# iamwinter/UMPR

Hardware: AMD Instinct MI355X
Metric: training samples/sec (higher is better)
Workload: dtype f32

## Files before the change

### umpr_amd/csrc/conv3x3.hip

```cpp
#include "umpr_common.h"
#include "umpr_internal.h"
#include "umpr_tiles.h"
#include <stdlib.h>
#include <type_traits>

namespace {

struct ConvParams {
  const float* x;
  const float* wm;
  const float* bias;
  const float* mask;
  float* y;
  int N, C, H, W, Cout, relu;
  long p0_base;
  long p_end;
};

template <int TM, int TN, bool BIAS, bool MASK, bool TAIL>
__device__ __forceinline__ void igemm_epilogue_as(const f32x16 (&tot)[TM][TN], const ConvParams& p, int HW, int row0,
                                                  const long (&obase)[TN], const bool (&pv)[TN]) {
  const int Cout = p.Cout;
  const bool relu = p.relu != 0;
  float bv[TM][16];
// ... 306 lines not shown
    okb = (okb & ~(1u << v)) | ((unsigned)ok << v);
  };
  auto store_a = [&](int v, int buf) {
    float* S = As[buf] + adst[v];
    S[0] = ra[v].x; S[LDA] = ra[v].y; S[2 * LDA] = ra[v].z; S[3 * LDA] = ra[v].w;
  };
  auto store_b = [&](int v, int buf) {
    const bool ok = (okb >> v) & 1;
    float* S = Ps[buf] + bdst[v];
    if (VEC == 4) *reinterpret_cast<float4*>(S) = ok ? rb[v] : make_float4(0.f, 0.f, 0.f, 0.f);
    else *reinterpret_cast<float2*>(S) = ok ? make_float2(rb[v].x, rb[v].y) : make_float2(0.f, 0.f);
  };
  constexpr int NPIECE = AV + BV;
  constexpr int KS = KC / 2;
  constexpr int ST0 = KS - NPIECE;
  static_assert(2 * NPIECE <= KS, "staging pieces must fit the k-steps of one stage");

#pragma unroll
  for (int v = 0; v < AV; ++v) load_a(v, 0);
#pragma unroll
  for (int v = 0; v < BV; ++v) load_b(v, 0);
#pragma unroll
  for (int v = 0; v < AV; ++v) store_a(v, 0);
#pragma unroll
  for (int v = 0; v < BV; ++v) store_b(v, 0);
  __syncthreads();
  for (int s0 = 0; s0 < ns; s0 += SFLUSH) {
#pragma unroll
    for (int i = 0; i < TM; ++i)
#pragma unroll
      for (int j = 0; j < TN; ++j)
#pragma unroll
        for (int r = 0; r < 16; ++r) acc[i][j][r] = 0.f;
    const int s1 = min(ns, s0 + SFLUSH);
    for (int s = s0; s < s1; ++s) {
      const int cur = s & 1;
      const int sn = min(s + 1, ns - 1);
      const float* as = As[cur] + half * LDA + wm * WTM + l31;
      const float* ps = Ps[cur];
      float a[2][TM], b[2][TN];
#pragma unroll
      for (int i = 0; i < TM; ++i) a[0][i] = as[i * 32];
#pragma unroll
      for (int j = 0; j < TN; ++j) b[0][j] = ps[boff[j]];
#pragma unroll
      for (int kk = 0; kk < KS; ++kk) {
        const int cb = kk & 1, nb = cb ^ 1;
        const int k1 = kk + 1, cl = k1 / 9, tap = k1 % 9;
#pragma unroll
        for (int m = 0; m < TM * TN; ++m) {
          const int i = m / TN, j = m % TN;
          acc[i][j] = mfma32(a[cb][i], b[cb][j], acc[i][j]);
          if (m == 0 && kk + 1 < KS) {
#pragma unroll
            for (int ii = 0; ii < TM; ++ii) a[nb][ii] = as[2 * k1 * LDA + ii * 32];
          }
          if (m == (TM * TN > 1 ? 1 : 0) && kk + 1 < KS) {
#pragma unroll
            for (int jj = 0; jj < TN; ++jj) b[nb][jj] = ps[boff[jj] + cl * PLANE + (tap / 3) * RW + (tap % 3)];
          }
          if (m == TM * TN - 1) {
            if (kk < AV) load_a(kk, sn);
            else if (kk < NPIECE) load_b(kk - AV, sn);
            else if (kk >= ST0 && kk - ST0 < AV) store_a(kk - ST0, cur ^ 1);
            else if (kk >= ST0 + AV) store_b(kk - ST0 - AV, cur ^ 1);
          }
          __builtin_amdgcn_sched_barrier(0);
        }
      }
      __syncthreads();
    }
#pragma unroll
    for (int i = 0; i < TM; ++i)
#pragma unroll
      for (int j = 0; j < TN; ++j) tot[i][j] += acc[i][j];
  }

  long obase[TN];
  bool pv[TN];
#pragma unroll
  for (int j = 0; j < TN; ++j) {
    const int d = wn * WTN + j * 32 + l31;
    pv[j] = d <= dlast;
    const int loc = yx0 + min(d, dlast);
    const int dn = loc / HW;
    obase[j] = (long)(n0 + dn) * p.Cout * HW + (loc - dn * HW);
  }
  igemm_epilogue<TM, TN>(tot, p, HW, m0 + __builtin_amdgcn_readfirstlane(wm) * WTM, half, obase, pv);
}

__global__ void pack_weights_kernel(const float* __restrict__ w, float* __restrict__ wp, int M, int C, int CinW,
                                    int transposed) {
  const int ns = (C + V2_CC - 1) / V2_CC;
  const long total = (long)M * ns * V2_KC;
  for (long i = blockIdx.x * (long)blockDim.x + threadIdx.x; i < total; i += (long)gridDim.x * blockDim.x) {
    const int kq = (int)(i % V2_KC);
    const long r = i / V2_KC;
    const int s = (int)(r % ns), m = (int)(r / ns);
    const int hf = kq & 1, j = kq >> 1;
    const int cl = j / 9, tap = j - cl * 9;
    const int c = s * V2_CC + cl + 2 * hf;
    float v = 0.f;
    if (c < C) v = transposed ? w[((long)c * CinW + m) * 9 + 8 - tap] : w[((long)m * CinW + c) * 9 + tap];
    wp[i] = v;
  }
}

constexpr int kSlots128 = 512;
template <int W>
void launch_v2(ConvParams p, int bn, hipStream_t s) {
  const long NP = (long)p.N * p.H * p.W;
  p.p0_base = 0; p.p_end = NP;
  if (p.Cout <= 64) {
    if (W >= 224 && bn != 128 && bn != 64) {
      const long ptiles = cdiv(NP, 256);
      dim3 grid((unsigned)(cdiv(ptiles, 8) * 8 * cdiv(p.Cout, 64)));
      conv3x3_igemm_v2_kernel<64, 256, W><<<grid, 256, 0, s>>>(p);
      return;
    }
    const long ptiles = cdiv(NP, 128);
    dim3 grid((unsigned)(cdiv(ptiles, 8) * 8 * cdiv(p.Cout, 64)));
    conv3x3_igemm_v2_kernel<64, 128, W><<<grid, 256, 0, s>>>(p);
    return;
  }
  const int mt = cdiv(p.Cout, 128);
  const long pt = cdiv(NP, 128);
  long pt_main = pt;
  if (bn == 64) pt_main = 0;
  else if (bn == 0 && pt * mt > kSlots128) {
    const long full = (pt * mt / kSlots128) * kSlots128;
    if (pt * mt - full > 0 && pt * mt - full <= kSlots128 * 3 / 4) pt_main = full / mt;
  }
  if (pt_main > 0) {
    ConvParams q = p;
    q.p_end = pt_main * 128 < NP ? pt_main * 128 : NP;
    dim3 grid((unsigned)(cdiv(pt_main, 8) * 8 * mt));
    conv3x3_igemm_v2_kernel<128, 128, W><<<grid, 256, 0, s>>>(q);
  }
  if (pt_main < pt) {
    ConvParams q = p;
    q.p0_base = pt_main * 128;
    dim3 grid((unsigned)(cdiv(cdiv(NP - q.p0_base, 64), 8) * 8 * mt));
    conv3x3_igemm_v2_kernel<128, 64, W><<<grid, 256, 0, s>>>(q);
  }
}

__global__ void flip_transpose_kernel(const float* __restrict__ w, float* __restrict__ wt, int Cout, int Cin) {
  const long total = (long)Cout * Cin * 9;
  for (long i = blockIdx.x * (long)blockDim.x + threadIdx.x; i < total; i += (long)gridDim.x * blockDim.x) {
    const int t = (int)(i % 9);
    const long r = i / 9;
    const int co = (int)(r % Cout), ci = (int)(r / Cout);
    wt[i] = w[((long)co * Cin + ci) * 9 + (8 - t)];
  }
}

struct WgradParams {
  const float* gz;
  const float* x;
  float* slab;
  float* bslab;
  int N, Cin, Cout, H, W;
  int R, CW;
  int segs_y, segs_x, nsegs, segs_per_split;
};

constexpr int WG_LDG = 33;
constexpr int WG_PLMAX = 103;

__global__ __launch_bounds__(256) void conv3x3_wgrad_kernel(WgradParams p) {
  __shared__ float Gs[2][64 * WG_LDG];
  __shared__ float Xs[2][64 * WG_PLMAX];
  __shared__ int pxoff[32];
  const int tid = threadIdx.x, lane = tid & 63, wave = tid >> 6;
  const int wm = wave >> 1, wn = wave & 1;
  const int l31 = lane & 31, kh = lane >> 5;
  const int co0 = blockIdx.y * 64, ci0 = blockIdx.x * 64;
  const int split = blockIdx.z;
  const int RW = p.CW + 2;
  const int patch = (p.R + 2) * RW;
  const int PL = patch | 1;
  const int npx = p.R * p.CW;
  const int HW = p.H * p.W;
  if (tid < 32) pxoff[tid] = tid < npx ? (tid / p.CW) * RW + (tid % p.CW) : 0;

  f32x16 acc[9];
#pragma unroll
  for (int t = 0; t < 9; ++t)
#pragma unroll
    for (int r = 0; r < 16; ++r) acc[t][r] = 0.f;
  float bsum[8];
#pragma unroll
  for (int v = 0; v < 8; ++v) bsum[v] = 0.f;

  const int sbeg = split * p.segs_per_split;
  const int send = min(p.nsegs, sbeg + p.segs_per_split);
  const int xs_total = 64 * patch;
  constexpr int XV = (64 * 102 + 255) / 256;
  float rg[8];
  float rx[XV];
  unsigned okg = 0, okx = 0;

  auto load = [&](int seg) {
    okg = 0; okx = 0;
    const int sx = seg % p.segs_x;
    const int sy = (seg / p.segs_x) % p.segs_y;
    const int n = seg / (p.segs_x * p.segs_y);
    const int y0 = sy * p.R, x0 = sx * p.CW;
#pragma unroll
    for (int v = 0; v < 8; ++v) {
      const int e = tid + v * 256;
      const int co = e >> 5, px = e & 31;
      const int r = px / p.CW, c = px - r * p.CW;
      const bool ok = px < npx && co0 + co < p.Cout && y0 + r < p.H && x0 + c < p.W;
      rg[v] = p.gz[ok ? ((long)n * p.Cout + co0 + co) * HW + (y0 + r) * p.W + x0 + c : 0];
      okg |= (unsigned)ok << v;
    }
#pragma unroll
    for (int v = 0; v < XV; ++v) {
      const int e = tid + v * 256;
      const int ci = e / patch, q = e - ci * patch;
      const int rr = q / RW, cc = q - rr * RW;
      const int yy = y0 - 1 + rr, xx = x0 - 1 + cc;
      const bool ok = e < xs_total && ci0 + ci < p.Cin && yy >= 0 && yy < p.H && xx >= 0 && xx < p.W;
      rx[v] = p.x[ok ? ((long)n * p.Cin + ci0 + ci) * HW + yy * p.W + xx : 0];
      okx |= (unsigned)ok << v;
    }
  };
  auto store = [&](int buf) {
#pragma unroll
    for (int v = 0; v < 8; ++v) {
      const int e = tid + v * 256;
      const float gv = ((okg >> v) & 1) ? rg[v] : 0.f;
      Gs[buf][(e >> 5) * WG_LDG + (e & 31)] = gv;
      if (p.bslab && blockIdx.x == 0) bsum[v] += gv;
    }
#pragma unroll
    for (int v = 0; v < XV; ++v) {
      const int e = tid + v * 256;
      if (e < xs_total) {
        const int ci = e / patch, q = e - ci * patch;
        Xs[buf][ci * PL + q] = ((okx >> v) & 1) ? rx[v] : 0.f;
      }
    }
  };

  if (sbeg < send) {
    load(sbeg);
    store(0);
  }
  __syncthreads();
  for (int s = sbeg; s < send; ++s) {
    const int cur = (s - sbeg) & 1;
    if (s + 1 < send) load(s + 1);
    const float* gs = Gs[cur] + (wm * 32 + l31) * WG_LDG;
    const float* xs = Xs[cur] + (wn * 32 + l31) * PL;
    float a[2], b[2][9];
    {
      a[0] = gs[kh];
      const float* xp = xs + pxoff[kh];
#pragma unroll
      for (int t = 0; t < 9; ++t) b[0][t] = xp[(t / 3) * RW + (t % 3)];
    }
#pragma unroll
    for (int kk = 0; kk < 16; ++kk) {
      const int cb = kk & 1, nb = cb ^ 1;
      if (kk + 1 < 16) {
        const int px = 2 * (kk + 1) + kh;
        a[nb] = gs[px];
        const float* xp = xs + pxoff[px];
#pragma unroll
        for (int t = 0; t < 9; ++t) b[nb][t] = xp[(t / 3) * RW + (t % 3)];
      }
      __builtin_amdgcn_sched_barrier(0);
#pragma unroll
      for (int t = 0; t < 9; ++t) acc[t] = mfma32(a[cb], b[cb][t], acc[t]);
      __builtin_amdgcn_sched_barrier(0);
    }
    if (s + 1 < send) store(cur ^ 1);
    __syncthreads();
  }

#pragma unroll
  for (int t = 0; t < 9; ++t) {
#pragma unroll
    for (int r = 0; r < 16; ++r) {
      const int co = co0 + wm * 32 + mfma_row(r, lane);
      const int ci = ci0 + wn * 32 + l31;
      if (co < p.Cout && ci < p.Cin) p.slab[(((long)split * 9 + t) * p.Cout + co) * p.Cin + ci] = acc[t][r];
    }
  }
  if (p.bslab && blockIdx.x == 0) {
#pragma unroll
    for (int v = 0; v < 8; ++v) {
      float sv = bsum[v];
#pragma unroll
      for (int o = 16; o > 0; o >>= 1) sv += __shfl_xor(sv, o, 64);
      const int co = co0 + (tid >> 5) + 8 * v;
      if ((tid & 31) == 0 && co < p.Cout) p.bslab[(long)split * p.Cout + co] = sv;
    }
  }
}

template <int R, int CW>
__global__ __launch_bounds__(256, 2) void conv3x3_wgrad_v2_kernel(WgradParams p) {
  constexpr int RW = CW + 2, PP = (R + 2) * RW, PL = PP | 1, NPX = R * CW;
  constexpr int G = 256 / PP;
  constexpr int CPG = (64 + G - 1) / G;
  static_assert((CW & 1) == 0 && NPX <= 32 && PP <= 102, "segment geometry");
  __shared__ float Gs[2][64 * WG_LDG];
  __shared__ float Xs[2][64 * PL];
  const int tid = threadIdx.x, lane = tid & 63, wave = tid >> 6;
  const int wm = wave >> 1, wn = wave & 1;
  const int l31 = lane & 31, kh = lane >> 5;
  const int co0 = blockIdx.y * 64, ci0 = blockIdx.x * 64;
  const int split = blockIdx.z;
  const int H = p.H, W = p.W, HW = H * W;

  const int pg = tid / PP, pos = tid - pg * PP;
  const bool pact = pg < G;
  const int prr = pos / RW, pcc = pos - prr * RW;
  const int gpx = tid & 31, gco = tid >> 5;
  const int gr = gpx / CW, gc = gpx - gr * CW;

  f32x16 acc[9];
#pragma unroll
  for (int t = 0; t < 9; ++t)
#pragma unroll
    for (int r = 0; r < 16; ++r) acc[t][r] = 0.f;
  float bsum[8];
#pragma unroll
  for (int v = 0; v < 8; ++v) bsum[v] = 0.f;

  const int sbeg = split * p.segs_per_split;
  const int send = min(p.nsegs, sbeg + p.segs_per_split);
  float rg[8];
  float rx[CPG];
  unsigned okg = 0, okx = 0;

  int cy0 = 0, cx0 = 0; long cgb = 0, cxb = 0; bool cgo = false, cxo = false;
  auto seg_setup = [&](int seg) {
    const int sx = seg % p.segs_x;
    const int sy = (seg / p.segs_x) % p.segs_y;
    const int n = seg / (p.segs_x * p.segs_y);
    cy0 = sy * R; cx0 = sx * CW;
    cgo = gpx < NPX && cy0 + gr < H && cx0 + gc < W;
    cgb = (((long)n * p.Cout + co0 + gco) * H + cy0 + gr) * W + cx0 + gc;
    const int yy = cy0 - 1 + prr, xx = cx0 - 1 + pcc;
    cxo = pact && yy >= 0 && yy < H && xx >= 0 && xx < W;
    cxb = (((long)n * p.Cin + ci0 + pg) * H + yy) * W + xx;
    okg = 0; okx = 0;
  };
  auto load_g = [&](int v) {
    const bool okv = cgo && co0 + gco + 8 * v < p.Cout;
    rg[v] = p.gz[okv ? cgb + (long)v * 8 * HW : 0];
    okg |= (unsigned)okv << v;
  };
  auto load_x = [&](int v) {
    const int ci = pg + G * v;
    const bool okv = cxo && ci < 64 && ci0 + ci < p.Cin;
    rx[v] = p.x[okv ? cxb + (long)v * G * HW : 0];
    okx |= (unsigned)okv << v;
  };
  auto store_g = [&](int v, int buf, bool fresh) {
    const float gv = ((okg >> v) & 1) ? rg[v] : 0.f;
    Gs[buf][(gco + 8 * v) * WG_LDG + gpx] = gv;
    bsum[v] += fresh ? gv : 0.f;
  };
  auto store_x = [&](int v, int buf) {
    const int ci = pg + G * v;
    if (pact && ci < 64) Xs[buf][ci * PL + pos] = ((okx >> v) & 1) ? rx[v] : 0.f;
  };
  constexpr int NP_ = 8 + CPG;
  constexpr int NSLOT = 16 * 9;
  static_assert(2 * NP_ <= NSLOT, "pieces must fit the MFMA slots of one segment");

  if (sbeg < send) {
    seg_setup(sbeg);
#pragma unroll
    for (int v = 0; v < 8; ++v) load_g(v);
#pragma unroll
    for (int v = 0; v < CPG; ++v) load_x(v);
#pragma unroll
    for (int v = 0; v < 8; ++v) store_g(v, 0, true);
#pragma unroll
    for (int v = 0; v < CPG; ++v) store_x(v, 0);
  }
  __syncthreads();
  for (int s = sbeg; s < send; ++s) {
    const int cur = (s - sbeg) & 1;
    const bool fresh = s + 1 < send;
    seg_setup(min(s + 1, send - 1));
    const float* gs = Gs[cur] + (wm * 32 + l31) * WG_LDG + kh;
    const float* xs = Xs[cur] + (wn * 32 + l31) * PL + kh;
    float a[2], b[2][9];
    a[0] = gs[0];
#pragma unroll
    for (int t = 0; t < 9; ++t) b[0][t] = xs[(t / 3) * RW + (t % 3)];
#pragma unroll
    for (int kk = 0; kk < 16; ++kk) {
      const int cb = kk & 1, nb = cb ^ 1;
      const int px = 2 * (kk + 1);
      const int po = px < NPX ? (px / CW) * RW + (px % CW) : 0;
#pragma unroll
      for (int t = 0; t < 9; ++t) {
        acc[t] = mfma32(a[cb], b[cb][t], acc[t]);
        if (kk + 1 < 16) {
          if (t == 0) a[nb] = gs[px];
          b[nb][t] = xs[po + (t / 3) * RW + (t % 3)];
        }
        const int q = kk * 9 + t;
        if (q < 8) load_g(q);
        else if (q < NP_) load_x(q - 8);
        else if (q >= NSLOT - NP_ && q < NSLOT - CPG) store_g(q - (NSLOT - NP_), cur ^ 1, fresh);
        else if (q >= NSLOT - CPG) store_x(q - (NSLOT - CPG), cur ^ 1);
        __builtin_amdgcn_sched_barrier(0);
      }
    }
    __syncthreads();
  }

#pragma unroll
  for (int t = 0; t < 9; ++t) {
#pragma unroll
    for (int r = 0; r < 16; ++r) {
      const int co = co0 + wm * 32 + mfma_row(r, lane);
      const int ci = ci0 + wn * 32 + l31;
      if (co < p.Cout && ci < p.Cin) p.slab[(((long)split * 9 + t) * p.Cout + co) * p.Cin + ci] = acc[t][r];
    }
  }
  if (p.bslab && blockIdx.x == 0) {
#pragma unroll
    for (int v = 0; v < 8; ++v) {
      float sv = bsum[v];
#pragma unroll
      for (int o = 16; o > 0; o >>= 1) sv += __shfl_xor(sv, o, 64);
      const int co = co0 + gco + 8 * v;
      if (gpx == 0 && co < p.Cout) p.bslab[(long)split * p.Cout + co] = sv;
    }
  }
}

template <int R, int CW>
__global__ __launch_bounds__(256) void conv3x3_wgrad_c3_kernel(WgradParams p) {
  constexpr int RW = CW + 2, PP = (R + 2) * RW, PL = PP | 1, NPX = R * CW;
  static_assert((CW & 1) == 0 && NPX <= 32 && PP <= 102, "segment geometry");
  __shared__ float Gs[2][64 * WG_LDG];
  __shared__ float Xs[2][4 * PL];
  __shared__ float Red[2][32 * 33];
  const int tid = threadIdx.x, lane = tid & 63, wave = tid >> 6;
  const int wm = wave & 1, wk = wave >> 1;
  const int l31 = lane & 31, kh = lane >> 5;
  const int co0 = blockIdx.y * 64;
  const int split = blockIdx.z;
  const int H = p.H, W = p.W, HW = H * W;
  const int gpx = tid & 31, gco = tid >> 5;
  const int gr = gpx / CW, gc = gpx - gr * CW;
  f32x16 acc;
#pragma unroll
  for (int r = 0; r < 16; ++r) acc[r] = 0.f;
  float bsum[8];
#pragma unroll
  for (int v = 0; v < 8; ++v) bsum[v] = 0.f;
  const int sbeg = split * p.segs_per_split;
  const int send = min(p.nsegs, sbeg + p.segs_per_split);
  float rg[8], rx[2];
  unsigned okg = 0, okx = 0;
  auto load = [&](int seg) {
    const int sx = seg % p.segs_x;
    const int sy = (seg / p.segs_x) % p.segs_y;
    const int n = seg / (p.segs_x * p.segs_y);
    const int y0 = sy * R, x0 = sx * CW;
    okg = 0; okx = 0;
    const bool ok = gpx < NPX && y0 + gr < H && x0 + gc < W;
    const long base = (((long)n * p.Cout + co0 + gco) * H + y0 + gr) * W + x0 + gc;
#pragma unroll
    for (int v = 0; v < 8; ++v) {
      const bool okv = ok && co0 + gco + 8 * v < p.Cout;
      rg[v] = p.gz[okv ? base + (long)v * 8 * HW : 0];
      okg |= (unsigned)okv << v;
    }
#pragma unroll
    for (int v = 0; v < 2; ++v) {
      const int e = tid + 256 * v;
      const int ci = e / PP, pos = e - ci * PP;
      const int prr = pos / RW, pcc = pos - prr * RW;
      const int yy = y0 - 1 + prr, xx = x0 - 1 + pcc;
      const bool okv = ci < p.Cin && yy >= 0 && yy < H && xx >= 0 && xx < W;
      rx[v] = p.x[okv ? (((long)n * p.Cin + ci) * H + yy) * W + xx : 0];
      okx |= (unsigned)okv << v;
    }
  };
  auto store = [&](int buf, bool fresh) {
#pragma unroll
    for (int v = 0; v < 8; ++v) {
      const float gv = ((okg >> v) & 1) ? rg[v] : 0.f;
      Gs[buf][(gco + 8 * v) * WG_LDG + gpx] = gv;
      bsum[v] += fresh ? gv : 0.f;
    }
#pragma unroll
    for (int v = 0; v < 2; ++v) {
      const int e = tid + 256 * v;
      const int ci = e / PP, pos = e - ci * PP;
      if (ci < 4) Xs[buf][ci * PL + pos] = ((okx >> v) & 1) ? rx[v] : 0.f;
    }
  };
  const int jc = l31 / 9, jt = l31 - jc * 9;
  const int xcol = (jc < 3 ? jc : 3) * PL + (jt / 3) * RW + (jt % 3) + kh;
  if (sbeg < send) { load(sbeg); store(0, true); }
  __syncthreads();
  for (int s = sbeg; s < send; ++s) {
    const int cur = (s - sbeg) & 1;
    load(min(s + 1, send - 1));
    const float* gs = Gs[cur] + (wm * 32 + l31) * WG_LDG + kh;
    const float* xs = Xs[cur] + xcol;
#pragma unroll
    for (int q = 0; q < 8; ++q) {
      const int kk = 2 * q + wk;
      const int px = 2 * kk;
      const int po = (px / CW) * RW + (px % CW);
      const int px0 = 2 * (2 * q), px1 = 2 * (2 * q + 1);
      const int po0 = (px0 / CW) * RW + (px0 % CW), po1 = (px1 / CW) * RW + (px1 % CW);
      const float a = wk ? gs[px1] : gs[px0];
      const float b = wk ? xs[po1] : xs[po0];
      (void)px; (void)po;
      acc = mfma32(a, b, acc);
    }
    store(cur ^ 1, s + 1 < send);
    __syncthreads();
  }
  if (wk == 1) {
#pragma unroll
    for (int r = 0; r < 16; ++r) Red[wm][mfma_row(r, lane) * 33 + l31] = acc[r];
  }
  __syncthreads();
  if (wk == 0) {
#pragma unroll
    for (int r = 0; r < 16; ++r) {
      const int row = mfma_row(r, lane);
      const float v = acc[r] + Red[wm][row * 33 + l31];
      const int co = co0 + wm * 32 + row;
      if (co < p.Cout && jc < p.Cin && l31 < 9 * p.Cin)
        p.slab[(((long)split * 9 + jt) * p.Cout + co) * p.Cin + jc] = v;
    }
  }
  if (p.bslab) {
#pragma unroll
    for (int v = 0; v < 8; ++v) {
      float sv = bsum[v];
#pragma unroll
      for (int o = 16; o > 0; o >>= 1) sv += __shfl_xor(sv, o, 64);
      const int co = co0 + gco + 8 * v;
      if (gpx == 0 && co < p.Cout) p.bslab[(long)split * p.Cout + co] = sv;
    }
  }
}

__global__ void wgrad_reduce_kernel(const float* __restrict__ slab, const float* __restrict__ bslab, int splits,
                                    int Cout, int Cin, float* __restrict__ dw, float* __restrict__ db, int accumulate) {
  const long per = (long)9 * Cout * Cin;
  const long total = per + (bslab ? Cout : 0);
  for (long i = blockIdx.x * (long)blockDim.x + threadIdx.x; i < total; i += (long)gridDim.x * blockDim.x) {
    if (i < per) {
      float v0 = 0.f, v1 = 0.f, v2 = 0.f, v3 = 0.f;
      int s = 0;
      for (; s + 3 < splits; s += 4) {
        v0 += slab[(long)s * per + i]; v1 += slab[(long)(s + 1) * per + i];
        v2 += slab[(long)(s + 2) * per + i]; v3 += slab[(long)(s + 3) * per + i];
      }
      for (; s < splits; ++s) v0 += slab[(long)s * per + i];
      const float v = (v0 + v1) + (v2 + v3);
      const int ci = (int)(i % Cin);
      const long r = i / Cin;
      const int co = (int)(r % Cout), t = (int)(r / Cout);
      float* d = dw + ((long)co * Cin + ci) * 9 + t;
      *d = accumulate ? *d + v : v;
    } else {
      const int co = (int)(i - per);
      float v = 0.f;
      for (int s = 0; s < splits; ++s) v += bslab[(long)s * Cout + co];
      db[co] = accumulate ? db[co] + v : v;
    }
  }
}

__global__ void maxpool2_fwd_kernel(const float* __restrict__ x, float* __restrict__ y, long planes, int H, int W) {
  const int Ho = H / 2, Wo = W / 2;
  const long total = planes * Ho * Wo;
  for (long i = blockIdx.x * (long)blockDim.x + threadIdx.x; i < total; i += (long)gridDim.x * blockDim.x) {
    const int xo = (int)(i % Wo);
    const long r = i / Wo;
    const int yo = (int)(r % Ho);
    const long pl = r / Ho;
    const float* s = x + (pl * H + 2 * yo) * W + 2 * xo;
    const float2 a = *reinterpret_cast<const float2*>(s);
    const float2 b = *reinterpret_cast<const float2*>(s + W);
    y[i] = fmaxf(fmaxf(a.x, a.y), fmaxf(b.x, b.y));
  }
}

__global__ void maxpool2_bwd_relu_kernel(const float* __restrict__ x, const float* __restrict__ gy,
                                         float* __restrict__ gx, long planes, int H, int W) {
  const int Ho = H / 2, Wo = W / 2;
  const long total = planes * Ho * Wo;
  for (long i = blockIdx.x * (long)blockDim.x + threadIdx.x; i < total; i += (long)gridDim.x * blockDim.x) {
    const int xo = (int)(i % Wo);
    const long r = i / Wo;
    const int yo = (int)(r % Ho);
    const long pl = r / Ho;
    const long o = (pl * H + 2 * yo) * W + 2 * xo;
    const float2 a = *reinterpret_cast<const float2*>(x + o);
    const float2 b = *reinterpret_cast<const float2*>(x + o + W);
    int arg = 0;
    float m = a.x;
    if (a.y > m) { m = a.y; arg = 1; }
    if (b.x > m) { m = b.x; arg = 2; }
    if (b.y > m) { m = b.y; arg = 3; }
    const float g = m > 0.f ? gy[i] : 0.f;
    float2 ga = make_float2(arg == 0 ? g : 0.f, arg == 1 ? g : 0.f);
    float2 gb = make_float2(arg == 2 ? g : 0.f, arg == 3 ? g : 0.f);
    *reinterpret_cast<float2*>(gx + o) = ga;
    *reinterpret_cast<float2*>(gx + o + W) = gb;
  }
}

}

static int conv_bn() { static const int v = umpr_env_int("UMPR_CONV_BN", 0); return v; }
template <int TM>
__global__ __launch_bounds__(256) void conv3x3_fwd_c3_kernel(ConvParams p) {
  constexpr int KS = 14;
  const int lane = threadIdx.x & 63, l31 = lane & 31, half = lane >> 5;
  const long wave = (long)blockIdx.x * 4 + (threadIdx.x >> 6);
  const long nwaves = (long)gridDim.x * 4;
  const int KR = p.C * 9;
  float wa[TM][KS];
#pragma unroll
  for (int i = 0; i < TM; ++i)
#pragma unroll
    for (int kk = 0; kk < KS; ++kk) {
      const int k = 2 * kk + half;
      wa[i][kk] = k < KR ? p.wm[(long)(i * 32 + l31) * KR + k] : 0.f;
    }
  float bv[TM][16];
#pragma unroll
  for (int i = 0; i < TM; ++i)
#pragma unroll
    for (int r = 0; r < 16; ++r) bv[i][r] = p.bias ? p.bias[i * 32 + mfma_row(r, lane)] : 0.f;
  const long HW = (long)p.H * p.W;
  const long ntiles = (p.p_end + 31) / 32;
  for (long t = wave; t < ntiles; t += nwaves) {
    const long px = t * 32 + l31;
    const bool okp = px < p.p_end;
    const long pc = okp ? px : 0;
    const int n = (int)(pc / HW);
    const int rem = (int)(pc - (long)n * HW);
    const int y = rem / p.W, x = rem - y * p.W;
    const float* img = p.x + (long)n * p.C * HW;
    float b[KS];
#pragma unroll
    for (int kk = 0; kk < KS; ++kk) {
      const int k = 2 * kk + half;
      const int c = k / 9, tap = k - c * 9;
      const int yy = y + tap / 3 - 1, xx = x + tap % 3 - 1;
      const bool ok = okp && k < KR && yy >= 0 && yy < p.H && xx >= 0 && xx < p.W;
      const float v = img[ok ? (long)c * HW + (long)yy * p.W + xx : 0];
      b[kk] = ok ? v : 0.f;
    }
    f32x16 acc[TM];
#pragma unroll
    for (int i = 0; i < TM; ++i)
#pragma unroll
      for (int r = 0; r < 16; ++r) acc[i][r] = bv[i][r];
#pragma unroll
    for (int kk = 0; kk < KS; ++kk)
#pragma unroll
      for (int i = 0; i < TM; ++i) acc[i] = mfma32(wa[i][kk], b[kk], acc[i]);
    if (okp) {
      float* out = p.y + (long)n * p.Cout * HW + rem;
#pragma unroll
      for (int i = 0; i < TM; ++i)
#pragma unroll
        for (int r = 0; r < 16; ++r) {
          float v = acc[i][r];
          if (p.relu) v = fmaxf(v, 0.f);
          out[(long)(i * 32 + mfma_row(r, lane)) * HW] = v;
        }
    }
  }
}

namespace {
struct ConvSwitches { bool wino, v1, wgrad_wino, w112, w112_fwd, v_reuse; int f4, c21_fwd; };
ConvSwitches read_conv_switches() {
  ConvSwitches v;
  v.wino = umpr_env_on("UMPR_CONV_WINO");
  v.v1 = umpr_env_int("UMPR_CONV_V1", 0) == 1;
  v.wgrad_wino = umpr_env_on("UMPR_WGRAD_WINO");
  v.f4 = umpr_env_int("UMPR_WINO_F4", 2);
  const int w112 = umpr_env_int("UMPR_WINO_112", -1);
  v.w112 = w112 == 1 || (w112 < 0 && v.f4 >= 1);
  v.w112_fwd = umpr_env_int("UMPR_WINO_112_FWD", 1) != 0;
  v.c21_fwd = umpr_env_int("UMPR_WINO_C21_FWD", -1);
  v.v_reuse = umpr_env_int("UMPR_WINO_V_REUSE", 1) != 0;
  return v;
}
const ConvSwitches& conv_switches() { static const ConvSwitches v = read_conv_switches(); return v; }

void wgrad_segment(int W, int* R, int* CW) {
  if (W % 16 == 0) { *R = 2; *CW = 16; }
  else if (W % 8 == 0) { *R = 4; *CW = 8; }
  else if (W % 14 == 0) { *R = 2; *CW = 14; }
  else if (W < 32) { *R = 32 / W; *CW = W; }
  else { *R = 1; *CW = 32; }
}

struct LayerClass { bool deep, c22, c21, f4_shape; };
LayerClass layer_class(int Cin, int Cout, int H, int W) {
  const bool at112 = conv_switches().w112 && H == 112 && W == 112;
  return {H == W && (W == 56 || W == 28 || W == 14), at112 && Cin >= 128 && Cout >= 128, at112 && Cin >= 64 && Cout >= 128,
          36L * ((H + 3) / 4) * ((W + 3) / 4) < 16L * (H / 2) * (W / 2)};
}

ConvAlgo direct_algo(ConvPass pass, int Cin, int Cout, int H, int W) {
  if (conv_switches().v1) return CONV_GENERIC;
  if (pass == CONV_WGRAD) {
    int R, CW;
    wgrad_segment(W, &R, &CW);
    if (R == 2 && CW == 16) return Cin <= 3 ? CONV_C3 : CONV_DIRECT;
    return (R == 4 && CW == 8) || (R == 2 && CW == 14) ? CONV_DIRECT : CONV_GENERIC;
  }
  if (pass == CONV_FWD && Cin <= 3 && Cout == 64) return CONV_C3;
  return H == W && (W == 224 || W == 112 || W == 56 || W == 28 || W == 14) ? CONV_DIRECT : CONV_GENERIC;
}

ConvAlgo conv_algo(ConvPass pass, int Cin, int Cout, int H, int W, bool inference) {
  const ConvSwitches& sw = conv_switches();
  const LayerClass lc = layer_class(Cin, Cout, H, W);
  bool wino, f4 = sw.f4 >= 1 && lc.f4_shape;
  if (pass == CONV_FWD) {
    const bool inf = inference && sw.f4 >= 1;
    const bool wide = inf || (sw.w112_fwd && sw.f4 >= 2);
    const bool c21 = lc.c21 && (sw.c21_fwd == 1 || (sw.c21_fwd < 0 && inf));
    wino = sw.wino && Cin >= 32 && (lc.deep || (wide && (lc.c22 || c21)));
    f4 = f4 && (inf || sw.f4 >= 2);
  } else if (pass == CONV_DGRAD) {
    wino = sw.wino && Cout >= 32 && (lc.deep || lc.c22);
  } else {
    wino = sw.wgrad_wino && Cin >= 32 && Cout >= 32 && (lc.deep || lc.c22 || lc.c21);
    f4 = f4 && (H % 4) == 0 && (W % 4) == 0;
  }
  if (!wino || sw.v1) return direct_algo(pass, Cin, Cout, H, W);
  return f4 ? CONV_WINO4 : CONV_WINO2;
}

constexpr int kWgradTargetWgs = 512;
struct WgradGeom { int R, CW, segs_y, segs_x, nsegs, splits, segs_per_split; size_t per_split, bytes; };
WgradGeom wgrad_geom(int N, int Cin, int Cout, int H, int W) {
  WgradGeom g;
  wgrad_segment(W, &g.R, &g.CW);
  g.segs_y = cdiv(H, g.R); g.segs_x = cdiv(W, g.CW); g.nsegs = N * g.segs_y * g.segs_x;
  g.splits = cdiv(kWgradTargetWgs, cdiv(Cout, 64) * cdiv(Cin, 64));
  if (g.splits > g.nsegs) g.splits = g.nsegs;
  g.segs_per_split = cdiv(g.nsegs, g.splits);
  g.per_split = ((size_t)9 * Cout * Cin + Cout) * sizeof(float);
  g.bytes = (size_t)g.splits * g.per_split;
  return g;
}
}

ConvPlan umpr_conv3x3_plan(ConvPass pass, int N, int Cin, int Cout, int H, int W, bool inference) {
  const ConvSwitches& sw = conv_switches();
  const LayerClass lc = layer_class(Cin, Cout, H, W);
  ConvPlan p;
  p.algo = conv_algo(pass, Cin, Cout, H, W, inference);
  p.direct = direct_algo(pass, Cin, Cout, H, W);
  p.edge = p.algo == CONV_WINO4 && ((H % 4) != 0 || (W % 4) != 0);
  p.v_floats = 0;
  const bool wino = p.algo == CONV_WINO2 || p.algo == CONV_WINO4;
  if (pass == CONV_WGRAD) {
    p.ws_floats = wino ? umpr_wino_wgrad_geom(N, Cin, Cout, H, W, p.algo == CONV_WINO4).floats
                       : wgrad_geom(N, Cin, Cout, H, W).bytes / sizeof(float);
  } else {
    const int M = pass == CONV_DGRAD ? Cin : Cout, C = pass == CONV_DGRAD ? Cout : Cin;
    p.ws_floats = (size_t)M * ((C + V2_CC - 1) / V2_CC) * V2_KC;
    const bool c21_possible = pass == CONV_FWD && lc.c21 && sw.c21_fwd != 0;
    if (sw.wino && (lc.deep || lc.c22 || c21_possible)) {
      const bool f4 = sw.f4 >= 1 && lc.f4_shape;
      size_t f = umpr_wino_conv_geom(N, C, M, H, W, f4).floats;
      if (f4 && pass == CONV_FWD) {
        const size_t f2 = umpr_wino_conv_geom(N, C, M, H, W, false).floats;
        if (f2 > f) f = f2;
      }
      if (f > p.ws_floats) p.ws_floats = f;
    }
  }
  if (pass != CONV_DGRAD && !(pass == CONV_FWD && inference) && sw.v_reuse &&
      conv_algo(CONV_FWD, Cin, Cout, H, W, false) == CONV_WINO4 && conv_algo(CONV_WGRAD, Cin, Cout, H, W, false) == CONV_WINO4) {
    const WinoConvGeom fg = umpr_wino_conv_geom(N, Cin, Cout, H, W, true);
    const WinoWgradGeom wg = umpr_wino_wgrad_geom(N, Cin, Cout, H, W, true);
    if (fg.v_floats == (size_t)wg.planes * wg.Cpad * wg.Tpad) p.v_floats = fg.v_floats;
  }
  return p;
}

size_t umpr_conv3x3_pack_floats(int N, int Cin, int Cout, int H, int W) {
  const size_t f = umpr_conv3x3_plan(CONV_FWD, N, Cin, Cout, H, W, false).ws_floats;
  const size_t t = umpr_conv3x3_plan(CONV_DGRAD, N, Cin, Cout, H, W, false).ws_floats;
  return f > t ? f : t;
}

bool umpr_conv3x3_pool_fold_ok(int N, int Cin, int Cout, int H, int W) {
  static const bool on = umpr_env_on("UMPR_POOL_FOLD");
  if (!on || (H % 2) != 0 || (W % 2) != 0) return false;
  const ConvAlgo wg = umpr_conv3x3_plan(CONV_WGRAD, N, Cin, Cout, H, W, false).algo;
  return umpr_conv3x3_plan(CONV_DGRAD, N, Cin, Cout, H, W, false).algo == CONV_WINO4 && (wg == CONV_WINO4 || wg == CONV_WINO2);
}

int umpr_conv3x3_run(const float* x, const float* w, int transposed, const float* bias, const float* mask, float* y,
                     int N, int Cin, int Cout, int H, int W, int relu, float* wpack, size_t wpack_floats,
                     const ConvHints& hints, hipStream_t s) {
  UMPR_REQUIRE(N > 0 && Cin > 0 && H > 0 && W > 0 && Cout > 0, "conv3x3: bad shape");
  UMPR_REQUIRE(transposed || !mask, "conv3x3: the forward pass takes no mask");
  const int M = transposed ? Cin : Cout;
  const int C = transposed ? Cout : Cin;
  const long NP = (long)N * H * W;
  const ConvPlan plan = umpr_conv3x3_plan(transposed ? CONV_DGRAD : CONV_FWD, N, Cin, Cout, H, W, hints.inference);
  ConvAlgo algo = plan.algo;
  const bool fits = wpack && wpack_floats >= plan.ws_floats;
  if (hints.v_slot)
    UMPR_REQUIRE(algo == CONV_WINO4 && fits && plan.v_floats > 0 && plan.v_floats == hints.v_slot_floats,
// ... 192 lines not shown
```

Measured before the change: 2188.

## Streamline wgrad kernel address math and deepen c3 prefetch pipeline

Replaces per-segment div/mod index recomputation with an incremental segment walker, and turns predicated loads into clamped unsigned offsets plus bitmask zeroing. In the c3 kernel, loads now run two segments ahead using double register stages, and the per-iteration wave-select branches are removed. The v2 kernel also batches B-operand LDS reads in groups of three and adds a fast unpredicated store path for full tiles. The tighter static_asserts restrict which geometries compile, and the extra register stage may raise register pressure.

```diff
diff --git a/umpr_amd/csrc/conv3x3.hip b/umpr_amd/csrc/conv3x3.hip
--- a/umpr_amd/csrc/conv3x3.hip
+++ b/umpr_amd/csrc/conv3x3.hip
@@ -632,12 +632,46 @@
   }
 }
 
+__device__ __forceinline__ float wg_keep(float v, unsigned m) { return __uint_as_float(__float_as_uint(v) & m); }
+
+struct WgSegWalk {
+  int sx, sy, y0, x0, segs_x, segs_y;
+  long gb, xb;
+  int step_x, step_row, R_, CW_;
+  long step_img_g, step_img_x;
+  __device__ __forceinline__ void init(const WgradParams& p, int R, int CW, int seg, int co0, int ci0) {
+    segs_x = p.segs_x; segs_y = p.segs_y; R_ = R; CW_ = CW;
+    sx = seg % segs_x;
+    const int t = seg / segs_x;
+    sy = t % segs_y;
+    const int n = t / segs_y;
+    y0 = sy * R; x0 = sx * CW;
+    gb = (((long)n * p.Cout + co0) * p.H + y0) * p.W + x0;
+    xb = (((long)n * p.Cin + ci0) * p.H + y0 - 1) * p.W + x0 - 1;
+    step_x = CW;
+    step_row = R * p.W - (segs_x - 1) * CW;
+    const long back = (long)(segs_y - 1) * R * p.W + (segs_x - 1) * CW;
+    step_img_g = (long)p.Cout * p.H * p.W - back;
+    step_img_x = (long)p.Cin * p.H * p.W - back;
+  }
+  __device__ __forceinline__ void advance(bool go) {
+    const bool cx = sx + 1 == segs_x, cy = cx && sy + 1 == segs_y;
+    const long dg = cy ? step_img_g : (long)(cx ? step_row : step_x);
+    const long dx = cy ? step_img_x : (long)(cx ? step_row : step_x);
+    const int nsx = cx ? 0 : sx + 1, nsy = cy ? 0 : (cx ? sy + 1 : sy);
+    gb += go ? dg : 0; xb += go ? dx : 0;
+    sx = go ? nsx : sx; sy = go ? nsy : sy;
+    y0 = sy * R_; x0 = sx * CW_;
+  }
+};
+
 template <int R, int CW>
 __global__ __launch_bounds__(256, 2) void conv3x3_wgrad_v2_kernel(WgradParams p) {
   constexpr int RW = CW + 2, PP = (R + 2) * RW, PL = PP | 1, NPX = R * CW;
   constexpr int G = 256 / PP;
   constexpr int CPG = (64 + G - 1) / G;
-  static_assert((CW & 1) == 0 && NPX <= 32 && PP <= 102, "segment geometry");
+  static_assert((CW & 1) == 0 && NPX <= 32 && PP <= 102 && PL == PP + 1, "segment geometry");
+  static_assert(G * (CPG - 1) < 64 && G * (CPG - 2) + G - 1 < 64, "only the last piece can pass channel 63");
   __shared__ float Gs[2][64 * WG_LDG];
   __shared__ float Xs[2][64 * PL];
   const int tid = threadIdx.x, lane = tid & 63, wave = tid >> 6;
@@ -652,6 +686,13 @@
   const int prr = pos / RW, pcc = pos - prr * RW;
   const int gpx = tid & 31, gco = tid >> 5;
   const int gr = gpx / CW, gc = gpx - gr * CW;
+  const int cin_t = p.Cin - ci0, cout_t = p.Cout - co0;
+  const unsigned gpo = (unsigned)(gr * W + gc), gch = (unsigned)(min(gco, cout_t - 1) * HW), glast = (unsigned)((cout_t - 1) * HW);
+  const unsigned xpo = (unsigned)(prr * W + pcc), xch = (unsigned)(min(min(pg, G - 1), cin_t - 1) * HW);
+  const unsigned xlast = (unsigned)((cin_t - 1) * HW);
+  const int gsw = gco * WG_LDG + gpx;
+  const int xsw = pact ? pg * PL + pos : PP;
+  const int xsw_last = pact && pg + G * (CPG - 1) < 64 ? (pg + G * (CPG - 1)) * PL + pos : PP;
 
   f32x16 acc[9];
 #pragma unroll
@@ -666,53 +707,38 @@
   const int send = min(p.nsegs, sbeg + p.segs_per_split);
   float rg[8];
   float rx[CPG];
-  unsigned okg = 0, okx = 0;
-
-  int cy0 = 0, cx0 = 0; long cgb = 0, cxb = 0; bool cgo = false, cxo = false;
-  auto seg_setup = [&](int seg) {
-    const int sx = seg % p.segs_x;
-    const int sy = (seg / p.segs_x) % p.segs_y;
-    const int n = seg / (p.segs_x * p.segs_y);
-    cy0 = sy * R; cx0 = sx * CW;
-    cgo = gpx < NPX && cy0 + gr < H && cx0 + gc < W;
-    cgb = (((long)n * p.Cout + co0 + gco) * H + cy0 + gr) * W + cx0 + gc;
-    const int yy = cy0 - 1 + prr, xx = cx0 - 1 + pcc;
-    cxo = pact && yy >= 0 && yy < H && xx >= 0 && xx < W;
-    cxb = (((long)n * p.Cin + ci0 + pg) * H + yy) * W + xx;
-    okg = 0; okx = 0;
+
+  WgSegWalk w;
+  w.init(p, R, CW, min(sbeg, p.nsegs - 1), co0, ci0);
+  unsigned gv = 0, gl = 0, xv = 0, xl = 0;
+  unsigned zg = 0, zx = 0, zb = 0;
+  auto seg_setup = [&](bool fresh) {
+    const bool cgo = (gpx < NPX) & (w.y0 + gr < H) & (w.x0 + gc < W);
+    const bool cxo = pact & ((unsigned)(w.y0 - 1 + prr) < (unsigned)H) & ((unsigned)(w.x0 - 1 + pcc) < (unsigned)W);
+    const unsigned g0 = cgo ? gpo : 0u;
+    const unsigned x0 = cxo ? xpo : (unsigned)(W + 1);
+    gv = g0 + gch; gl = g0 + glast; xv = x0 + xch; xl = x0 + xlast;
+    zg = cgo ? ~0u : 0u; zx = cxo ? ~0u : 0u; zb = fresh ? zg : 0u;
   };
-  auto load_g = [&](int v) {
-    const bool okv = cgo && co0 + gco + 8 * v < p.Cout;
-    rg[v] = p.gz[okv ? cgb + (long)v * 8 * HW : 0];
-    okg |= (unsigned)okv << v;
+  auto load_g = [&](int v) { rg[v] = (p.gz + w.gb)[min(gv + (unsigned)(v * 8 * HW), gl)]; };
+  auto load_x = [&](int v) { rx[v] = (p.x + w.xb)[min(xv + (unsigned)(v * G * HW), xl)]; };
+  auto store_g = [&](int v, int buf) {
+    Gs[buf][gsw + 8 * v * WG_LDG] = wg_keep(rg[v], zg);
+    bsum[v] += wg_keep(rg[v], zb);
   };
-  auto load_x = [&](int v) {
-    const int ci = pg + G * v;
-    const bool okv = cxo && ci < 64 && ci0 + ci < p.Cin;
-    rx[v] = p.x[okv ? cxb + (long)v * G * HW : 0];
-    okx |= (unsigned)okv << v;
-  };
-  auto store_g = [&](int v, int buf, bool fresh) {
-    const float gv = ((okg >> v) & 1) ? rg[v] : 0.f;
-    Gs[buf][(gco + 8 * v) * WG_LDG + gpx] = gv;
-    bsum[v] += fresh ? gv : 0.f;
-  };
-  auto store_x = [&](int v, int buf) {
-    const int ci = pg + G * v;
-    if (pact && ci < 64) Xs[buf][ci * PL + pos] = ((okx >> v) & 1) ? rx[v] : 0.f;
-  };
+  auto store_x = [&](int v, int buf) { Xs[buf][v < CPG - 1 ? xsw + v * G * PL : xsw_last] = wg_keep(rx[v], zx); };
   constexpr int NP_ = 8 + CPG;
   constexpr int NSLOT = 16 * 9;
   static_assert(2 * NP_ <= NSLOT, "pieces must fit the MFMA slots of one segment");
 
   if (sbeg < send) {
-    seg_setup(sbeg);
+    seg_setup(true);
 #pragma unroll
     for (int v = 0; v < 8; ++v) load_g(v);
 #pragma unroll
     for (int v = 0; v < CPG; ++v) load_x(v);
 #pragma unroll
-    for (int v = 0; v < 8; ++v) store_g(v, 0, true);
+    for (int v = 0; v < 8; ++v) store_g(v, 0);
 #pragma unroll
     for (int v = 0; v < CPG; ++v) store_x(v, 0);
   }
@@ -720,7 +746,8 @@
   for (int s = sbeg; s < send; ++s) {
     const int cur = (s - sbeg) & 1;
     const bool fresh = s + 1 < send;
-    seg_setup(min(s + 1, send - 1));
+    w.advance(fresh);
+    seg_setup(fresh);
     const float* gs = Gs[cur] + (wm * 32 + l31) * WG_LDG + kh;
     const float* xs = Xs[cur] + (wn * 32 + l31) * PL + kh;
     float a[2], b[2][9];
@@ -736,13 +763,16 @@
       for (int t = 0; t < 9; ++t) {
         acc[t] = mfma32(a[cb], b[cb][t], acc[t]);
         if (kk + 1 < 16) {
-          if (t == 0) a[nb] = gs[px];
-          b[nb][t] = xs[po + (t / 3) * RW + (t % 3)];
+          if (t == 1) a[nb] = gs[px];
+          if (t % 3 == 0) {
+#pragma unroll
+            for (int u = 0; u < 3; ++u) b[nb][t + u] = xs[po + (t / 3) * RW + u];
+          }
         }
         const int q = kk * 9 + t;
         if (q < 8) load_g(q);
         else if (q < NP_) load_x(q - 8);
-        else if (q >= NSLOT - NP_ && q < NSLOT - CPG) store_g(q - (NSLOT - NP_), cur ^ 1, fresh);
+        else if (q >= NSLOT - NP_ && q < NSLOT - CPG) store_g(q - (NSLOT - NP_), cur ^ 1);
         else if (q >= NSLOT - CPG) store_x(q - (NSLOT - CPG), cur ^ 1);
         __builtin_amdgcn_sched_barrier(0);
       }
@@ -750,13 +780,23 @@
     __syncthreads();
   }
 
-#pragma unroll
-  for (int t = 0; t < 9; ++t) {
-#pragma unroll
-    for (int r = 0; r < 16; ++r) {
-      const int co = co0 + wm * 32 + mfma_row(r, lane);
-      const int ci = ci0 + wn * 32 + l31;
-      if (co < p.Cout && ci < p.Cin) p.slab[(((long)split * 9 + t) * p.Cout + co) * p.Cin + ci] = acc[t][r];
+  const bool full = co0 + 64 <= p.Cout && ci0 + 64 <= p.Cin;
+  const int ci = ci0 + wn * 32 + l31;
+  if (full) {
+#pragma unroll
+    for (int t = 0; t < 9; ++t) {
+      float* o = p.slab + (((long)split * 9 + t) * p.Cout + co0 + wm * 32) * p.Cin + ci;
+#pragma unroll
+      for (int r = 0; r < 16; ++r) o[(long)mfma_row(r, lane) * p.Cin] = acc[t][r];
+    }
+  } else {
+#pragma unroll
+    for (int t = 0; t < 9; ++t) {
+#pragma unroll
+      for (int r = 0; r < 16; ++r) {
+        const int co = co0 + wm * 32 + mfma_row(r, lane);
+        if (co < p.Cout && ci < p.Cin) p.slab[(((long)split * 9 + t) * p.Cout + co) * p.Cin + ci] = acc[t][r];
+      }
     }
   }
   if (p.bslab && blockIdx.x == 0) {
@@ -774,7 +814,7 @@
 template <int R, int CW>
 __global__ __launch_bounds__(256) void conv3x3_wgrad_c3_kernel(WgradParams p) {
   constexpr int RW = CW + 2, PP = (R + 2) * RW, PL = PP | 1, NPX = R * CW;
-  static_assert((CW & 1) == 0 && NPX <= 32 && PP <= 102, "segment geometry");
+  static_assert((CW & 3) == 0 && NPX <= 32 && PP <= 102 && PL == PP + 1, "segment geometry");
   __shared__ float Gs[2][64 * WG_LDG];
   __shared__ float Xs[2][4 * PL];
   __shared__ float Red[2][32 * 33];
@@ -786,6 +826,21 @@
   const int H = p.H, W = p.W, HW = H * W;
   const int gpx = tid & 31, gco = tid >> 5;
   const int gr = gpx / CW, gc = gpx - gr * CW;
+  const int cout_t = p.Cout - co0;
+  const unsigned gpo = (unsigned)(gr * W + gc), gch = (unsigned)(min(gco, cout_t - 1) * HW), glast = (unsigned)((cout_t - 1) * HW);
+  const int gsw = gco * WG_LDG + gpx;
+  int prr[2], pcc[2], xsw[2];
+  unsigned xvo[2];
+  bool pact[2];
+#pragma unroll
+  for (int v = 0; v < 2; ++v) {
+    const int e = tid + 256 * v;
+    const int ci = e / PP, pos = e - ci * PP;
+    prr[v] = pos / RW; pcc[v] = pos - prr[v] * RW;
+    pact[v] = ci < 4;
+    xvo[v] = (unsigned)((min(ci, p.Cin - 1) * H + prr[v]) * W + pcc[v]);
+    xsw[v] = pact[v] ? ci * PL + pos : PP;
+  }
   f32x16 acc;
 #pragma unroll
   for (int r = 0; r < 16; ++r) acc[r] = 0.f;
@@ -794,69 +849,69 @@
   for (int v = 0; v < 8; ++v) bsum[v] = 0.f;
   const int sbeg = split * p.segs_per_split;
   const int send = min(p.nsegs, sbeg + p.segs_per_split);
-  float rg[8], rx[2];
-  unsigned okg = 0, okx = 0;
-  auto load = [&](int seg) {
-    const int sx = seg % p.segs_x;
-    const int sy = (seg / p.segs_x) % p.segs_y;
-    const int n = seg / (p.segs_x * p.segs_y);
-    const int y0 = sy * R, x0 = sx * CW;
-    okg = 0; okx = 0;
-    const bool ok = gpx < NPX && y0 + gr < H && x0 + gc < W;
-    const long base = (((long)n * p.Cout + co0 + gco) * H + y0 + gr) * W + x0 + gc;
+  struct Stage { float rg[8], rx[2]; unsigned zg, zx[2]; };
+  Stage st[2];
+  WgSegWalk w;
+  w.init(p, R, CW, min(sbeg, p.nsegs - 1), co0, 0);
+  int wseg = sbeg;
+  auto load = [&](Stage& d) {
+    const bool cgo = (gpx < NPX) & (w.y0 + gr < H) & (w.x0 + gc < W);
+    const unsigned g0 = cgo ? gpo : 0u;
+    d.zg = cgo ? ~0u : 0u;
+#pragma unroll
+    for (int v = 0; v < 8; ++v) d.rg[v] = (p.gz + w.gb)[min(g0 + gch + (unsigned)(v * 8 * HW), g0 + glast)];
+#pragma unroll
+    for (int v = 0; v < 2; ++v) {
+      const bool cxo = pact[v] & ((unsigned)(w.y0 - 1 + prr[v]) < (unsigned)H) & ((unsigned)(w.x0 - 1 + pcc[v]) < (unsigned)W);
+      d.zx[v] = cxo ? ~0u : 0u;
+      d.rx[v] = (p.x + w.xb)[cxo ? xvo[v] : (unsigned)(W + 1)];
+    }
+  };
+  auto next_seg = [&]() {
+    const bool go = wseg + 1 < send;
+    w.advance(go);
+    wseg += go ? 1 : 0;
+  };
+  auto store = [&](const Stage& d, int buf, bool fresh) {
+    const unsigned zb = fresh ? d.zg : 0u;
 #pragma unroll
     for (int v = 0; v < 8; ++v) {
-      const bool okv = ok && co0 + gco + 8 * v < p.Cout;
-      rg[v] = p.gz[okv ? base + (long)v * 8 * HW : 0];
-      okg |= (unsigned)okv << v;
-    }
-#pragma unroll
-    for (int v = 0; v < 2; ++v) {
-      const int e = tid + 256 * v;
-      const int ci = e / PP, pos = e - ci * PP;
-      const int prr = pos / RW, pcc = pos - prr * RW;
-      const int yy = y0 - 1 + prr, xx = x0 - 1 + pcc;
-      const bool okv = ci < p.Cin && yy >= 0 && yy < H && xx >= 0 && xx < W;
-      rx[v] = p.x[okv ? (((long)n * p.Cin + ci) * H + yy) * W + xx : 0];
-      okx |= (unsigned)okv << v;
-    }
-  };
-  auto store = [&](int buf, bool fresh) {
-#pragma unroll
-    for (int v = 0; v < 8; ++v) {
-      const float gv = ((okg >> v) & 1) ? rg[v] : 0.f;
-      Gs[buf][(gco + 8 * v) * WG_LDG + gpx] = gv;
-      bsum[v] += fresh ? gv : 0.f;
-    }
-#pragma unroll
-    for (int v = 0; v < 2; ++v) {
-      const int e = tid + 256 * v;
-      const int ci = e / PP, pos = e - ci * PP;
-      if (ci < 4) Xs[buf][ci * PL + pos] = ((okx >> v) & 1) ? rx[v] : 0.f;
-    }
+      Gs[buf][gsw + 8 * v * WG_LDG] = wg_keep(d.rg[v], d.zg);
+      bsum[v] += wg_keep(d.rg[v], zb);
+    }
+#pragma unroll
+    for (int v = 0; v < 2; ++v) Xs[buf][xsw[v]] = wg_keep(d.rx[v], d.zx[v]);
   };
   const int jc = l31 / 9, jt = l31 - jc * 9;
-  const int xcol = (jc < 3 ? jc : 3) * PL + (jt / 3) * RW + (jt % 3) + kh;
-  if (sbeg < send) { load(sbeg); store(0, true); }
+  const int xcol = (jc < 3 ? jc : 3) * PL + (jt / 3) * RW + (jt % 3) + kh + 2 * wk;
+  const int gcol = (wm * 32 + l31) * WG_LDG + kh + 2 * wk;
+  auto mma = [&](int cur) {
+    const float* gs = Gs[cur] + gcol;
+    const float* xs = Xs[cur] + xcol;
+#pragma unroll
+    for (int q = 0; q < 8; ++q) {
+      const int px = 4 * q;
+      acc = mfma32(gs[px], xs[(px / CW) * RW + (px % CW)], acc);
+    }
+  };
+  if (sbeg < send) {
+    load(st[0]);
+    store(st[0], 0, true);
+    next_seg();
+    load(st[0]);
+  }
   __syncthreads();
-  for (int s = sbeg; s < send; ++s) {
-    const int cur = (s - sbeg) & 1;
-    load(min(s + 1, send - 1));
-    const float* gs = Gs[cur] + (wm * 32 + l31) * WG_LDG + kh;
-    const float* xs = Xs[cur] + xcol;
-#pragma unroll
-    for (int q = 0; q < 8; ++q) {
-      const int kk = 2 * q + wk;
-      const int px = 2 * kk;
-      const int po = (px / CW) * RW + (px % CW);
-      const int px0 = 2 * (2 * q), px1 = 2 * (2 * q + 1);
-      const int po0 = (px0 / CW) * RW + (px0 % CW), po1 = (px1 / CW) * RW + (px1 % CW);
-      const float a = wk ? gs[px1] : gs[px0];
-      const float b = wk ? xs[po1] : xs[po0];
-      (void)px; (void)po;
-      acc = mfma32(a, b, acc);
-    }
-    store(cur ^ 1, s + 1 < send);
+  for (int s = sbeg; s < send; s += 2) {
+    next_seg();
+    load(st[1]);
+    mma(0);
+    store(st[0], 1, s + 1 < send);
+    __syncthreads();
+    if (s + 1 >= send) break;
+    next_seg();
+    load(st[0]);
+    mma(1);
+    store(st[1], 0, s + 2 < send);
     __syncthreads();
   }
   if (wk == 1) {
```

Result: no change. 2206 (median of 6 runs) (+0.8%).
